# yvokeller/Show-Attend-and-Tell

Hardware: AMD Instinct MI355X
Metric: train images/sec on COCO batch=128 at 1/2/4/8 MI355X (higher is better)
Workload: dtype bf16; 1 GPU; COCO-shaped resnet152 encoder (bf16 fwd) + attention/tf/ado decoder train step, V=10000, T=27; global_batch=128, per_gpu_batch=128, seq_len=27, parallelism=dp1, hip_graph=True, encoder_decoder_overlap=True

## Files before the change

### include/sat_hip.h

```cpp
#ifndef SAT_HIP_H_
#define SAT_HIP_H_

#include <stddef.h>
#include <stdint.h>

#ifdef __cplusplus
extern "C" {
#endif

#define SAT_ABI_VERSION 9

enum { SAT_F32 = 0, SAT_BF16 = 1 };
enum { SAT_ACT_NONE = 0, SAT_ACT_RELU = 1, SAT_ACT_TANH = 2, SAT_ACT_SIGMOID = 3 };
enum { SAT_OK = 0, SAT_ERR_INVALID = 9001 };

typedef struct {
  int N, H, W, C, KH, KW, stride, pad, OH, OW;
} SatConvGeom;

typedef struct {
  int conv_pipe;
  int conv_stream;
  int conv3x3_ws;
  int conv_slices;
// ... 189 lines not shown
                            void* workspace, size_t workspace_bytes, int32_t* out_ids, int* out_len,
                            float* out_alphas, int* out_alpha_rows, float* out_score, void* stream);

size_t sat_decoder_beam_batch_workspace_bytes(const SatDecoderDims* d, int n_images, int beam_size, int max_step);
int sat_decoder_beam_search_batch(const SatDecoderDims* d, const SatDecoderLayout* lay, const float* params,
                                  const void* params_lp, const void* img_features, int n_images, int beam_size,
                                  int max_step, void* workspace, size_t workspace_bytes, int32_t* out_ids,
                                  int* out_len, float* out_alphas, int* out_alpha_rows, float* out_score,
                                  void* stream);

size_t sat_caption_loss_workspace_bytes(int B, int T, int L);
int sat_caption_loss_forward(int B, int T, int V, int L, int dtype, const void* preds,
                             const float* alphas, const int64_t* captions, float alpha_c,
                             int pad_id, int skip0, int skip1, int skip2, void* workspace,
                             float* out, void* stream);
int sat_caption_loss_forward_loss_out(int B, int T, int V, int L, int dtype, const void* preds,
                                      const float* alphas, const int64_t* captions, float alpha_c,
                                      int pad_id, int skip0, int skip1, int skip2, void* workspace,
                                      float* out, float* loss_out, void* stream);
int sat_caption_loss_backward(int B, int T, int V, int L, int dtype, const void* preds,
                              const int64_t* captions, float alpha_c, void* workspace,
                              const float* grad_out, void* d_preds, float* d_alphas, void* stream);
int sat_caption_loss_backward_relu(int B, int T, int V, int L, int dtype, const void* preds,
                              const int64_t* captions, float alpha_c, void* workspace,
                              const float* grad_out, void* d_preds, float* d_alphas, void* stream);
int sat_caption_loss_backward_ld(int B, int T, int V, int L, int dtype, const void* preds,
                                 const int64_t* captions, float alpha_c, void* workspace,
                                 const float* grad_out, void* d_preds, int64_t ld_dpreds,
                                 float* d_alphas, int relu_mask, void* stream);
size_t sat_caption_loss_weighted_workspace_bytes(int B, int T, int L);
int sat_caption_loss_weighted_forward(int B, int T, int V, int L, int dtype, const void* preds,
                                      const float* alphas, const int32_t* targets, const float* weights,
                                      float alpha_c, void* workspace, float* out, float* loss_out, float* logp,
                                      void* stream);
int sat_caption_loss_weighted_backward(int B, int T, int V, int L, int dtype, const void* preds,
                                       const int32_t* targets, const float* weights, void* workspace,
                                       const float* grad_out, void* d_preds, int64_t ld_dpreds, float* d_alphas,
                                       int relu_mask, void* stream);

enum { SAT_IMG_NCHW = 0, SAT_IMG_NHWC = 1, SAT_IMG_S2D16 = 2 };
size_t sat_images_workspace_bytes(int B, int OH, int OW);
int sat_images_max_downscale(void);
size_t sat_images_lds_bytes(int max_h, int max_w, int OH, int OW);
size_t sat_images_lds_limit(void);
int sat_images_to_input(const uint8_t* pixels, const int64_t* offsets, const int32_t* sizes, int B, int max_h,
                        int max_w, int OH, int OW, const float* mean, const float* std, int layout, int c_pad,
                        int dtype, void* out, void* workspace, size_t workspace_bytes, void* stream);

int sat_rows_gather(const void* table, int64_t n_rows, int64_t row_elems, int dtype, const int64_t* idx, int n,
                    void* out, int32_t* n_bad, void* stream);
int sat_rows_scatter(const void* src, int n, int64_t row_elems, int dtype, const int64_t* idx, void* table,
                     int64_t n_rows, int32_t* n_bad, void* stream);

int sat_cider_table_insert(uint32_t* table, int64_t slots, const uint32_t* keys, const float* values, int64_t n,
                           int32_t* n_bad, void* stream);
int sat_cider_lookup(const uint32_t* table, int64_t slots, float log_n, const uint32_t* keys, int64_t n, float* out,
                     void* stream);
int sat_cider_ref_norms(const uint32_t* table, int64_t slots, float log_n, const int32_t* ref_words,
                        const int32_t* ref_len, int n_refs, int ref_stride, float* ref_norm, void* stream);
int sat_cider_score(const uint32_t* table, int64_t slots, float log_n, const int32_t* ref_words,
                    const int32_t* ref_len, const float* ref_norm, int n_refs, int ref_stride,
                    const int32_t* img_ref_begin, int n_images, const int32_t* tokens, const int64_t* image, int n,
                    int T1, int start_id, int end_id, int pad_id, float* out, int32_t* n_bad, void* stream);

int sat_adam_step(float* param, const float* grad, float* exp_avg, float* exp_avg_sq,
                  void* param_lp, int64_t n, float beta1, float beta2, float eps,
                  float step_size, float bias_correction2_sqrt, void* stream);

#ifdef __cplusplus
}
#endif
#endif
```

### show-attend-and-tell_amd/_lib.py

```python
import ctypes
import os

import torch

_HERE = os.path.dirname(os.path.abspath(__file__))
LIB_PATH = os.environ.get("SAT_HIP_LIB_TUNING") or os.path.join(_HERE, "libsat_hip.so")

SAT_F32, SAT_BF16 = 0, 1
IMG_NCHW, IMG_NHWC, IMG_S2D16 = 0, 1, 2
ACT_NONE, ACT_RELU, ACT_TANH, ACT_SIGMOID = 0, 1, 2, 3

c_int, c_int64, c_float, c_void_p, c_size_t, c_uint64 = (ctypes.c_int, ctypes.c_int64, ctypes.c_float,
                                                        ctypes.c_void_p, ctypes.c_size_t, ctypes.c_uint64)


class SatConvGeom(ctypes.Structure):
    _fields_ = [(n, c_int) for n in ("N", "H", "W", "C", "KH", "KW", "stride", "pad", "OH", "OW")]


ABI_VERSION = 9


class SatPolicy(ctypes.Structure):
    _fields_ = [(n, c_int) for n in ("conv_pipe", "conv_stream", "conv3x3_ws", "conv_slices", "skinny", "gemm_stages",
# ... 137 lines not shown
    ("sat_decoder_forward_sample", c_int, [ctypes.POINTER(SatDecoderDims), ctypes.POINTER(SatDecoderLayout),
                                           c_void_p, c_void_p, c_void_p, c_void_p, c_void_p, c_float, c_void_p,
                                           c_void_p, c_size_t, c_void_p, c_void_p, c_void_p, c_void_p, c_void_p]),
    ("sat_sample_noise", c_int, [ctypes.POINTER(SatDecoderDims), c_int, c_int, c_int, c_void_p, c_void_p]),
    ("sat_decoder_backward", c_int, [ctypes.POINTER(SatDecoderDims), ctypes.POINTER(SatDecoderLayout), c_void_p,
                                     c_void_p, c_void_p, c_void_p, c_size_t, c_void_p, c_void_p, c_void_p,
                                     c_void_p, c_void_p, c_int, c_int, c_void_p]),
    ("sat_decoder_backward_features", c_int, [ctypes.POINTER(SatDecoderDims), ctypes.POINTER(SatDecoderLayout),
                                              c_void_p, c_void_p, c_void_p, c_void_p, c_size_t, c_void_p, c_void_p,
                                              c_void_p, c_void_p, c_void_p, c_int, c_int, c_void_p, c_void_p,
                                              c_void_p, c_size_t]),
    ("sat_decoder_feature_grad_workspace_bytes", c_size_t, [ctypes.POINTER(SatDecoderDims)]),
    ("sat_feature_grad_accumulate", c_int, [c_int, c_int, c_int, c_int, c_int, c_void_p, c_int64, c_int64, c_void_p,
                                            c_int64, c_int64, c_void_p, c_int64, c_void_p, c_int64, c_void_p,
                                            c_int64, c_void_p]),
    ("sat_decoder_step_bench", c_int, [ctypes.POINTER(SatDecoderDims), ctypes.POINTER(SatDecoderLayout), c_void_p,
                                       c_void_p, c_void_p, c_void_p, c_size_t, c_void_p, c_void_p, c_int, c_void_p,
                                       c_void_p]),
    ("sat_decoder_beam_workspace_bytes", c_size_t, [ctypes.POINTER(SatDecoderDims), c_int]),
    ("sat_decoder_beam_search", c_int, [ctypes.POINTER(SatDecoderDims), ctypes.POINTER(SatDecoderLayout), c_void_p,
                                        c_void_p, c_void_p, c_int, c_int, c_void_p, c_size_t, c_void_p, c_void_p,
                                        c_void_p, c_void_p, c_void_p, c_void_p]),
    ("sat_decoder_beam_batch_workspace_bytes", c_size_t, [ctypes.POINTER(SatDecoderDims), c_int, c_int, c_int]),
    ("sat_decoder_beam_search_batch", c_int, [ctypes.POINTER(SatDecoderDims), ctypes.POINTER(SatDecoderLayout),
                                              c_void_p, c_void_p, c_void_p, c_int, c_int, c_int, c_void_p, c_size_t,
                                              c_void_p, c_void_p, c_void_p, c_void_p, c_void_p, c_void_p]),
    ("sat_caption_loss_workspace_bytes", c_size_t, [c_int, c_int, c_int]),
    ("sat_caption_loss_forward", c_int, [c_int, c_int, c_int, c_int, c_int, c_void_p, c_void_p, c_void_p, c_float,
                                         c_int, c_int, c_int, c_int, c_void_p, c_void_p, c_void_p]),
    ("sat_caption_loss_forward_loss_out", c_int, [c_int, c_int, c_int, c_int, c_int, c_void_p, c_void_p, c_void_p,
                                                  c_float, c_int, c_int, c_int, c_int, c_void_p, c_void_p, c_void_p,
                                                  c_void_p]),
    ("sat_caption_loss_backward", c_int, [c_int, c_int, c_int, c_int, c_int, c_void_p, c_void_p, c_float,
                                          c_void_p, c_void_p, c_void_p, c_void_p, c_void_p]),
    ("sat_caption_loss_backward_relu", c_int, [c_int, c_int, c_int, c_int, c_int, c_void_p, c_void_p, c_float,
                                          c_void_p, c_void_p, c_void_p, c_void_p, c_void_p]),
    ("sat_caption_loss_backward_ld", c_int, [c_int, c_int, c_int, c_int, c_int, c_void_p, c_void_p, c_float,
                                             c_void_p, c_void_p, c_void_p, c_int64, c_void_p, c_int, c_void_p]),
    ("sat_caption_loss_weighted_workspace_bytes", c_size_t, [c_int, c_int, c_int]),
    ("sat_caption_loss_weighted_forward", c_int, [c_int, c_int, c_int, c_int, c_int, c_void_p, c_void_p, c_void_p,
                                                  c_void_p, c_float, c_void_p, c_void_p, c_void_p, c_void_p,
                                                  c_void_p]),
    ("sat_caption_loss_weighted_backward", c_int, [c_int, c_int, c_int, c_int, c_int, c_void_p, c_void_p, c_void_p,
                                                   c_void_p, c_void_p, c_void_p, c_int64, c_void_p, c_int, c_void_p]),
    ("sat_images_workspace_bytes", c_size_t, [c_int, c_int, c_int]),
    ("sat_images_max_downscale", c_int, []),
    ("sat_images_lds_bytes", c_size_t, [c_int, c_int, c_int, c_int]),
    ("sat_images_lds_limit", c_size_t, []),
    ("sat_images_to_input", c_int, [c_void_p, c_void_p, c_void_p, c_int, c_int, c_int, c_int, c_int,
                                    ctypes.POINTER(c_float), ctypes.POINTER(c_float), c_int, c_int, c_int, c_void_p,
                                    c_void_p, c_size_t, c_void_p]),
    ("sat_rows_gather", c_int, [c_void_p, c_int64, c_int64, c_int, c_void_p, c_int, c_void_p, c_void_p, c_void_p]),
    ("sat_rows_scatter", c_int, [c_void_p, c_int, c_int64, c_int, c_void_p, c_void_p, c_int64, c_void_p, c_void_p]),
    ("sat_cider_table_insert", c_int, [c_void_p, c_int64, c_void_p, c_void_p, c_int64, c_void_p, c_void_p]),
    ("sat_cider_lookup", c_int, [c_void_p, c_int64, c_float, c_void_p, c_int64, c_void_p, c_void_p]),
    ("sat_cider_ref_norms", c_int, [c_void_p, c_int64, c_float, c_void_p, c_void_p, c_int, c_int, c_void_p,
                                    c_void_p]),
    ("sat_cider_score", c_int, [c_void_p, c_int64, c_float, c_void_p, c_void_p, c_void_p, c_int, c_int, c_void_p,
                                c_int, c_void_p, c_void_p, c_int, c_int, c_int, c_int, c_int, c_void_p, c_void_p,
                                c_void_p]),
    ("sat_adam_step", c_int, [c_void_p, c_void_p, c_void_p, c_void_p, c_void_p, c_int64, c_float, c_float,
                              c_float, c_float, c_float, c_void_p]),
]
EXPORTED = [s[0] for s in _SIGNATURES]

_lib = None


def lib():
    global _lib
    if _lib is None:
        if not os.path.exists(LIB_PATH):
            raise RuntimeError(f"sat_amd: HIP library not found at {LIB_PATH}; build it with "
                               "`python -c 'import __graft_entry__ as g; g.build()'` (make -C "
                               "show-attend-and-tell_amd/csrc)")
        handle = ctypes.CDLL(LIB_PATH)
        for name, res, args in _SIGNATURES:
            fn = getattr(handle, name)
            fn.restype = res
            fn.argtypes = args
        version = handle.sat_abi_version()
        if version != ABI_VERSION:
            raise RuntimeError(f"sat_amd: {LIB_PATH} has C-ABI version {version}, this package binds version "
                               f"{ABI_VERSION}; rebuild it (make -C show-attend-and-tell_amd/csrc)")
        _lib = handle
    return _lib


def check(code, what):
    if code != 0:
        msg = lib().sat_error_string(code)
        raise RuntimeError(f"sat_amd: {what} failed with code {code}: {msg.decode() if msg else '?'}")


def dtype_code(dt):
    if dt == torch.float32:
        return SAT_F32
    if dt == torch.bfloat16:
        return SAT_BF16
    raise TypeError(f"sat_amd: unsupported dtype {dt} (float32 or bfloat16)")


def require_device(*tensors):
    for t in tensors:
        if t is not None and t.device.type != "cuda":
            raise RuntimeError("sat_amd: tensors must live on a HIP device (the product path has no CPU fallback)")
# ... 13 lines not shown
```

### show-attend-and-tell_amd/csrc/elementwise.hip

```cpp
#include "sat_common.h"
#include "sat_internal.h"

namespace {

constexpr int kMaxGrid = 2048;
inline int grid_for(long n, int per_block = 256) {
  long g = (n + per_block - 1) / per_block;
  return (int)(g < 1 ? 1 : (g > kMaxGrid ? kMaxGrid : g));
}

template <typename T>
__global__ void nchw_to_nhwc_kernel(const float* __restrict__ x, T* __restrict__ y, int N, int C, int H, int W,
                                    int Cp) {
  long total = (long)N * H * W;
  for (long p = blockIdx.x * (long)blockDim.x + threadIdx.x; p < total; p += (long)gridDim.x * blockDim.x) {
    long n = p / ((long)H * W), hw = p - n * H * W;
    const float* src = x + n * C * H * W + hw;
    T* dst = y + p * Cp;
    if (Cp * sizeof(T) == 16) {
      uint4 u;
      T* h = (T*)&u;
#pragma unroll
      for (int c = 0; c < 16 / (int)sizeof(T); ++c) h[c] = (T)(c < C ? src[(long)c * H * W] : 0.f);
      *(uint4*)dst = u;
// ... 356 lines not shown
      for (long i = blockIdx.x * (long)blockDim.x + threadIdx.x; i < R * C; i += stride) {
        const long r = i / C;
        p[r * ld + (i - r * C)] = 0.f;
      }
    }
  }
}

template <typename T>
__global__ void embed_gather_kernel(const float* __restrict__ W, const int32_t* __restrict__ tok, int R,
                                    long tok_stride_b, int T1, int E, T* __restrict__ out, long out_ld) {
  int r = blockIdx.x;
  if (r >= R) return;
  int b = r / T1, t = r - b * T1;
  int id = tok[(long)b * tok_stride_b + t];
  const float* src = W + (long)id * E;
  T* dst = out + (long)r * out_ld;
  for (int e = threadIdx.x; e < E; e += blockDim.x) dst[e] = (T)src[e];
}

template <typename OT>
__global__ void embed_gather_captions_kernel(const float* __restrict__ W, const int64_t* __restrict__ caps, int R,
                                             int T, int T1, int E, OT* __restrict__ out, long out_ld,
                                             int32_t* __restrict__ tok) {
  const int r = blockIdx.x;
  if (r >= R) return;
  const int b = r / T1, t = r - b * T1;
  const int id = (int)caps[(long)b * T + t];
  if (threadIdx.x == 0) tok[r] = id;
  const float* src = W + (long)id * E;
  OT* dst = out + (long)r * out_ld;
  if ((E & 3) == 0 && ((uintptr_t)src & 15) == 0) {
    for (int e = 4 * threadIdx.x; e < E; e += 4 * blockDim.x) {
      const float4 v = *(const float4*)(src + e);
      dst[e] = (OT)v.x; dst[e + 1] = (OT)v.y; dst[e + 2] = (OT)v.z; dst[e + 3] = (OT)v.w;
    }
  } else {
    for (int e = threadIdx.x; e < E; e += blockDim.x) dst[e] = (OT)src[e];
  }
}

__global__ void embed_scatter_kernel(const float* __restrict__ dX, const int32_t* __restrict__ tok, int R, int E,
                                     float* __restrict__ G) {
  int r = blockIdx.x;
  if (r >= R) return;
  int id = tok[r];
  const float* src = dX + (long)r * E;
  float* dst = G + (long)id * E;
  for (int e = threadIdx.x; e < E; e += blockDim.x) atomicAdd(dst + e, src[e]);
}

constexpr int kEmbSortMax = 16384, kEmbPiece = 32;
constexpr int kRankRows = 16, kRankParts = 16;
__global__ __launch_bounds__(256) void embed_rank_kernel(const int32_t* __restrict__ tok, int R,
                                                         int32_t* __restrict__ perm, int32_t* __restrict__ stok,
                                                         int32_t* __restrict__ seg) {
  __shared__ __attribute__((aligned(16))) int32_t st[kEmbSortMax];
  __shared__ int cnt[3][kRankParts][kRankRows];
  const int R4 = (R + 3) & ~3;
  for (int i = threadIdx.x; i < R4; i += blockDim.x) st[i] = i < R ? tok[i] : 0x7fffffff;
  __syncthreads();
  const int rl = threadIdx.x & (kRankRows - 1), part = threadIdx.x / kRankRows;
  const int r = blockIdx.x * kRankRows + rl;
  const int k = r < R ? st[r] : 0;
  const int words = R4 / 4, per = (words + kRankParts - 1) / kRankParts;
  const int w0 = part * per, w1 = min(words, w0 + per);
  int less = 0, before = 0, eq = 0;
#pragma unroll 4
  for (int wi = w0; wi < w1; ++wi) {
    const int i = 4 * wi;
    const int4 x = *(const int4*)(st + i);
    less += (x.x < k) + (x.y < k) + (x.z < k) + (x.w < k);
    eq += (x.x == k) + (x.y == k) + (x.z == k) + (x.w == k);
    before += ((x.x == k) & (i < r)) + ((x.y == k) & (i + 1 < r)) + ((x.z == k) & (i + 2 < r)) + ((x.w == k) & (i + 3 < r));
  }
  cnt[0][part][rl] = less; cnt[1][part][rl] = eq; cnt[2][part][rl] = before;
  __syncthreads();
  if (part != 0 || r >= R) return;
  for (int q = 1; q < kRankParts; ++q) { less += cnt[0][q][rl]; eq += cnt[1][q][rl]; before += cnt[2][q][rl]; }
  const int pos = less + before;
  perm[pos] = r;
  stok[pos] = k;
  seg[2 * pos] = less;
  seg[2 * pos + 1] = less + eq;
}

__global__ __launch_bounds__(64) void embed_segsum_kernel(const float* __restrict__ dX, int E,
                                                          const int32_t* __restrict__ perm,
                                                          const int32_t* __restrict__ stok,
                                                          const int32_t* __restrict__ seg, int R, float* G,
                                                          float* __restrict__ part, int accumulate) {
  const int p = blockIdx.x, e = blockIdx.y * 256 + 4 * threadIdx.x;
  const int s0 = p * kEmbPiece, n = min(R - s0, kEmbPiece);
  __shared__ int sr[kEmbPiece], stk[kEmbPiece], sa[kEmbPiece], sb[kEmbPiece];
  if ((int)threadIdx.x < n) {
    sr[threadIdx.x] = perm[s0 + threadIdx.x];
    stk[threadIdx.x] = stok[s0 + threadIdx.x];
    sa[threadIdx.x] = seg[2 * (s0 + threadIdx.x)];
    sb[threadIdx.x] = seg[2 * (s0 + threadIdx.x) + 1];
  }
  __syncthreads();
  if (e >= E) return;
  float4 x[kEmbPiece];
#pragma unroll
  for (int i = 0; i < kEmbPiece; ++i)
    x[i] = i < n ? *(const float4*)(dX + (long)sr[i] * E + e) : make_float4(0.f, 0.f, 0.f, 0.f);
  float4 acc = make_float4(0.f, 0.f, 0.f, 0.f);
  int rs = 0;
#pragma unroll
  for (int i = 0; i < kEmbPiece; ++i) {
    if (i < n) {
      acc = f4add(acc, x[i]);
      if (i + 1 == n || stk[i + 1] != stk[i]) {
        if (sa[i] == s0 + rs && sb[i] == s0 + i + 1) {
          float4* g = (float4*)(G + (long)stk[i] * E + e);
          *g = accumulate ? f4add(*g, acc) : acc;
        } else {
          *(float4*)(part + ((long)p * 2 + (rs == 0 ? 0 : 1)) * E + e) = acc;
        }
        acc = make_float4(0.f, 0.f, 0.f, 0.f);
        rs = i + 1;
      }
    }
  }
}

__global__ __launch_bounds__(256) void embed_segfix_kernel(const int32_t* __restrict__ stok,
                                                           const int32_t* __restrict__ seg, int R, int E,
                                                           const float* __restrict__ part, float* G,
                                                           int accumulate) {
  const int p = blockIdx.x, chain = threadIdx.x >> 6, e = blockIdx.y * 256 + 4 * (threadIdx.x & 63);
  const int s0 = p * kEmbPiece, s1 = min(R, s0 + kEmbPiece);
  const int sa = seg[2 * (s1 - 1)], sb = seg[2 * (s1 - 1) + 1];
  if (sb <= s1 || sa < s0) return;
  __shared__ float4 cs[3][64];
  const int p1 = (sb - 1) / kEmbPiece;
  float4 acc = make_float4(0.f, 0.f, 0.f, 0.f);
  if (e < E) {
    for (int q0 = p + 1 + chain; q0 <= p1; q0 += 32) {
      float4 y[8];
#pragma unroll
      for (int u = 0; u < 8; ++u) {
        const int q = q0 + 4 * u;
        y[u] = q <= p1 ? *(const float4*)(part + (long)q * 2 * E + e) : make_float4(0.f, 0.f, 0.f, 0.f);
      }
#pragma unroll
      for (int u = 0; u < 8; ++u) acc = f4add(acc, y[u]);
    }
  }
  if (chain > 0) cs[chain - 1][threadIdx.x & 63] = acc;
  __syncthreads();
  if (chain != 0 || e >= E) return;
  const float4 own = *(const float4*)(part + ((long)p * 2 + (sa == s0 ? 0 : 1)) * E + e);
  const float4 sum = f4add(own, f4add(f4add(acc, cs[0][threadIdx.x]), f4add(cs[1][threadIdx.x], cs[2][threadIdx.x])));
  float4* g = (float4*)(G + (long)stok[s1 - 1] * E + e);
  *g = accumulate ? f4add(*g, sum) : sum;
}

__device__ __forceinline__ bool am_better(float x, int xi, float y, int yi) { return sat_argmax_better(x, xi, y, yi); }
// ... 288 lines not shown
    else hipLaunchKernelGGL((argmax_kernel<bf16, false, true>), dim3(B), dim3(256), 0, s, (const bf16*)X, ld, V, out, out_stride, emb, E, (bf16*)emb_out, emb_ld, pre, pre_stride);
  } else {
    if (vec) hipLaunchKernelGGL((argmax_kernel<float, true, true>), dim3(B), dim3(256), 0, s, (const float*)X, ld, V, out, out_stride, emb, E, (float*)emb_out, emb_ld, pre, pre_stride);
    else hipLaunchKernelGGL((argmax_kernel<float, false, true>), dim3(B), dim3(256), 0, s, (const float*)X, ld, V, out, out_stride, emb, E, (float*)emb_out, emb_ld, pre, pre_stride);
  }
  return (int)hipGetLastError();
}

int sat_argmax_rows_sample(const void* X, int dtype, long ld, int B, int V, int32_t* out, long out_stride,
                           int32_t* out2, long out2_stride, const float* emb, int E, void* emb_out, long emb_ld,
                           const SatSampleArgs& sa, hipStream_t s) {
  if (V >= (1 << 20) || sa.t < 0 || sa.t >= (1 << 20)) return (int)hipErrorInvalidValue;
  const int esz = dtype == SAT_BF16 ? 2 : 4;
  const bool vec = ((uintptr_t)X & 15) == 0 && (ld * esz) % 16 == 0;
  if (dtype == SAT_BF16) {
    if (vec) hipLaunchKernelGGL((argmax_kernel<bf16, true, false, true>), dim3(B), dim3(256), 0, s, (const bf16*)X, ld, V, out, out_stride, emb, E, (bf16*)emb_out, emb_ld, nullptr, 0, sa, out2, out2_stride);
    else hipLaunchKernelGGL((argmax_kernel<bf16, false, false, true>), dim3(B), dim3(256), 0, s, (const bf16*)X, ld, V, out, out_stride, emb, E, (bf16*)emb_out, emb_ld, nullptr, 0, sa, out2, out2_stride);
  } else {
    if (vec) hipLaunchKernelGGL((argmax_kernel<float, true, false, true>), dim3(B), dim3(256), 0, s, (const float*)X, ld, V, out, out_stride, emb, E, (float*)emb_out, emb_ld, nullptr, 0, sa, out2, out2_stride);
    else hipLaunchKernelGGL((argmax_kernel<float, false, false, true>), dim3(B), dim3(256), 0, s, (const float*)X, ld, V, out, out_stride, emb, E, (float*)emb_out, emb_ld, nullptr, 0, sa, out2, out2_stride);
  }
  return (int)hipGetLastError();
}

int sat_cast_launch(const void* x, int xd, void* y, int yd, long n, hipStream_t s) {
  if (n <= 0) return 0;
  int g = grid_for(n);
  if (xd == SAT_F32 && yd == SAT_BF16) hipLaunchKernelGGL((cast_kernel<float, bf16>), dim3(g), dim3(256), 0, s, (const float*)x, (bf16*)y, n);
  else if (xd == SAT_BF16 && yd == SAT_F32) hipLaunchKernelGGL((cast_kernel<bf16, float>), dim3(g), dim3(256), 0, s, (const bf16*)x, (float*)y, n);
  else if (xd == SAT_F32) hipLaunchKernelGGL((cast_kernel<float, float>), dim3(g), dim3(256), 0, s, (const float*)x, (float*)y, n);
  else hipLaunchKernelGGL((cast_kernel<bf16, bf16>), dim3(g), dim3(256), 0, s, (const bf16*)x, (bf16*)y, n);
  return (int)hipGetLastError();
}

extern "C" int sat_abi_version(void) { return SAT_ABI_VERSION; }

extern "C" const char* sat_error_string(int code) {
  if (code == 0) return "success";
  if (code == SAT_ERR_INVALID) return "invalid argument or unsupported shape";
  return hipGetErrorString((hipError_t)code);
}

extern "C" int sat_cast(const void* x, int x_dtype, void* y, int y_dtype, int64_t n, void* stream) {
  SAT_REQUIRE(x && y && n >= 0);
  return sat_cast_launch(x, x_dtype, y, y_dtype, n, (hipStream_t)stream);
}

extern "C" int sat_mean_rows_abi(const void* a, int B, int L, int D, int dtype, float* out_f32, void* out_t,
                                 void* stream) {
  SAT_REQUIRE(a && B > 0 && L > 0 && D > 0);
  return sat_mean_rows(a, B, L, D, dtype, out_f32, out_t, (hipStream_t)stream);
}

extern "C" int sat_nchw_to_nhwc(int N, int C, int H, int W, int Cp, int dtype, const float* x, void* y,
                                void* stream) {
  SAT_REQUIRE(x && y && Cp >= C && C > 0);
  long pix = (long)N * H * W;
  int g = grid_for(pix);
  if (dtype == SAT_BF16)
    hipLaunchKernelGGL(nchw_to_nhwc_kernel<bf16>, dim3(g), dim3(256), 0, (hipStream_t)stream, x, (bf16*)y, N, C, H, W, Cp);
  else
    hipLaunchKernelGGL(nchw_to_nhwc_kernel<float>, dim3(g), dim3(256), 0, (hipStream_t)stream, x, (float*)y, N, C, H, W, Cp);
  return (int)hipGetLastError();
}

extern "C" int sat_nchw_to_s2d(int N, int C, int H, int W, int dtype, const float* x, void* y, void* stream) {
  SAT_REQUIRE(x && y && C > 0 && 4 * C <= 16 && H % 2 == 0 && W % 2 == 0);
  const int g = grid_for((long)N * (H / 2) * (W / 2));
  if (dtype == SAT_BF16 && C == 3 && ((uintptr_t)x & 7) == 0 && ((uintptr_t)y & 15) == 0) {
    const long total = (long)N * (H / 2) * (W / 2);
    hipLaunchKernelGGL(nchw3_to_s2d16_bf16_kernel, dim3((unsigned)((total + 255) / 256)), dim3(256), 0,
                       (hipStream_t)stream, x, (bf16*)y, N, H, W);
  } else if (dtype == SAT_BF16)
    hipLaunchKernelGGL(nchw_to_s2d16_kernel<bf16>, dim3(g), dim3(256), 0, (hipStream_t)stream, x, (bf16*)y, N, C, H, W);
  else
    hipLaunchKernelGGL(nchw_to_s2d16_kernel<float>, dim3(g), dim3(256), 0, (hipStream_t)stream, x, (float*)y, N, C, H, W);
  return (int)hipGetLastError();
}

extern "C" int sat_maxpool2d_nhwc(int N, int H, int W, int C, int k, int stride, int pad, int dtype, const void* x,
                                  void* y, int OH, int OW, void* stream) {
  SAT_REQUIRE(x && y && k > 0 && stride > 0);
  SAT_REQUIRE(OH == (H + 2 * pad - k) / stride + 1 && OW == (W + 2 * pad - k) / stride + 1);
  SAT_REQUIRE(C % 8 == 0 && ((uintptr_t)x & 15) == 0 && ((uintptr_t)y & 15) == 0);
  long total = (long)N * OH * OW * (C / 8);
  int g = grid_for(total);
  if (dtype == SAT_BF16 && k == 3) {
    hipLaunchKernelGGL(maxpool_bf16_kernel<3>, dim3((unsigned)((total + 255) / 256)), dim3(256), 0,
                       (hipStream_t)stream, (const bf16*)x, (bf16*)y, N, H, W, C, stride, pad, OH, OW);
  } else if (dtype == SAT_BF16)
    hipLaunchKernelGGL(maxpool_kernel<bf16>, dim3(g), dim3(256), 0, (hipStream_t)stream, (const bf16*)x, (bf16*)y, N, H,
                       W, C, k, stride, pad, OH, OW);
  else
    hipLaunchKernelGGL(maxpool_kernel<float>, dim3(g), dim3(256), 0, (hipStream_t)stream, (const float*)x, (float*)y, N,
                       H, W, C, k, stride, pad, OH, OW);
  return (int)hipGetLastError();
}

extern "C" int sat_adam_step(float* param, const float* grad, float* exp_avg, float* exp_avg_sq, void* param_lp,
                             int64_t n, float beta1, float beta2, float eps, float step_size,
                             float bias_correction2_sqrt, void* stream) {
  SAT_REQUIRE(param && grad && exp_avg && exp_avg_sq && n >= 0);
  constexpr int64_t kChunk = 1L << 28;
  for (int64_t i = 0; i < n; i += kChunk) {
    const int64_t m = n - i < kChunk ? n - i : kChunk;
    hipLaunchKernelGGL(adam_kernel, dim3(grid_for((m + 3) / 4)), dim3(256), 0, (hipStream_t)stream, param + i, grad + i,
// ... 7 lines not shown
```

### show-attend-and-tell_amd/csrc/loss.hip

```cpp
#include "sat_common.h"
#include "sat_internal.h"

namespace {

constexpr int kStat = 5;

__device__ __forceinline__ float block_sum(float v, float* red) {
  const int lane = threadIdx.x & 63, w = threadIdx.x >> 6, nw = blockDim.x >> 6;
  v = wave_sum(v);
  __syncthreads();
  if (lane == 0) red[w] = v;
  __syncthreads();
  float s = 0.f;
  for (int i = 0; i < nw; ++i) s += red[i];
  return s;
}
__device__ __forceinline__ float block_max(float v, float* red) {
  const int lane = threadIdx.x & 63, w = threadIdx.x >> 6, nw = blockDim.x >> 6;
  v = wave_max(v);
  __syncthreads();
  if (lane == 0) red[w] = v;
  __syncthreads();
  float s = -INFINITY;
  for (int i = 0; i < nw; ++i) s = fmaxf(s, red[i]);
// ... 147 lines not shown
    constexpr int LU = 4;
    const int NV = V / VEC;
    for (int c0 = threadIdx.x; c0 < NV; c0 += LU * 256) {
      uint4 u[LU];
#pragma unroll
      for (int k = 0; k < LU; ++k) {
        const int c = c0 + k * 256;
        u[k] = c < NV ? *(const uint4*)(x + (long)c * VEC) : make_uint4(0u, 0u, 0u, 0u);
      }
#pragma unroll
      for (int k = 0; k < LU; ++k) {
        const int c = c0 + k * 256;
        if (c >= NV) break;
        const TT* h = (const TT*)&u[k];
#pragma unroll
        for (int j = 0; j < VEC; ++j) {
          const float xv = (float)h[j];
          const int v = c * VEC + j;
          online_add(m, se, xv);
          cnt += (xv > xt || (xv == xt && v < tgt)) ? 1.f : 0.f;
        }
      }
    }
  } else {
    for (int v = threadIdx.x; v < V; v += blockDim.x) {
      const float xv = (float)x[v];
      online_add(m, se, xv);
      cnt += (xv > xt || (xv == xt && v < tgt)) ? 1.f : 0.f;
    }
  }
#pragma unroll
  for (int o = 32; o > 0; o >>= 1) {
    const float om = __shfl_xor(m, o, 64), os = __shfl_xor(se, o, 64);
    const float nm = fmaxf(m, om);
    se = (nm == -INFINITY) ? 0.f : se * expf(m - nm) + os * expf(om - nm);
    m = nm;
    cnt += __shfl_xor(cnt, o, 64);
  }
  const int lane = threadIdx.x & 63, w = threadIdx.x >> 6;
  if (lane == 0) { red_m[w] = m; red_s[w] = se; red_c[w] = cnt; }
  __syncthreads();
  if (threadIdx.x == 0) {
    float M = red_m[0], S = red_s[0], C = red_c[0];
    for (int i = 1; i < 4; ++i) {
      const float nm = fmaxf(M, red_m[i]);
      S = (nm == -INFINITY) ? 0.f : S * expf(M - nm) + red_s[i] * expf(red_m[i] - nm);
      M = nm;
      C += red_c[i];
    }
    write_stats(M + logf(S), xt, C);
  }
}

__global__ __launch_bounds__(256) void loss_reg_kernel(const float* __restrict__ alphas, int B, int T1, int L,
                                                       float alpha_c, float* __restrict__ dreg,
                                                       float* __restrict__ part) {
  __shared__ float red[4];
  const int i = blockIdx.x * blockDim.x + threadIdx.x;
  const float inv_bl = 1.0f / (float)(B * L);
  float reg = 0.f;
  if (i < B * L) {
    const int b = i / L, l = i - b * L;
    float ssum = 0.f;
    for (int t = 0; t < T1; ++t) ssum += alphas[((long)b * T1 + t) * L + l];
    const float d = 1.f - ssum;
    reg = d * d;
    dreg[i] = alpha_c * 2.f * (ssum - 1.f) * inv_bl;
  }
  reg = block_sum(reg, red);
  if (threadIdx.x == 0) part[blockIdx.x] = reg;
}

__global__ __launch_bounds__(1024) void loss_reduce_kernel(const float* __restrict__ stats, const float* __restrict__ part,
                                                           int nparts, const int64_t* __restrict__ caps, int B, int T,
                                                           int L, float alpha_c, int s0, int s1, int s2,
                                                           float* __restrict__ out, float* __restrict__ loss_out) {
  __shared__ float red[16];
  const int T1 = T - 1, R = B * T1;
  float ce = 0.f, c1 = 0.f, c5 = 0.f, np = 0.f;
  for (int r = threadIdx.x; r < R; r += blockDim.x) {
    const float* st = stats + (long)r * kStat;
    ce += st[1]; c1 += st[2]; c5 += st[3]; np += st[4];
  }
  ce = block_sum(ce, red);
  c1 = block_sum(c1, red);
  c5 = block_sum(c5, red);
  np = block_sum(np, red);
  float reg = 0.f;
  for (int i = threadIdx.x; i < nparts; i += blockDim.x) reg += part[i];
  reg = block_sum(reg, red);
  float cl = 0.f;
  for (int i = threadIdx.x; i < B * T; i += blockDim.x) {
    const int64_t tok = caps[i];
    cl += (tok != s0 && tok != s1 && tok != s2) ? 1.f : 0.f;
  }
  cl = block_sum(cl, red);
  if (threadIdx.x == 0) {
    const float cem = ce / (float)(B * (T1 - 1));
    const float regm = alpha_c * (reg * (1.0f / (float)(B * L)));
    out[0] = cem + regm;
    if (loss_out) loss_out[0] = cem + regm;
    out[1] = cem;
    out[2] = regm;
    out[3] = c1; out[4] = c5; out[5] = np; out[6] = cl;
  }
}

__global__ __launch_bounds__(1024) void wloss_reduce_kernel(const float* __restrict__ stats, const float* __restrict__ part,
                                                            int nparts, int R, int BL, float alpha_c,
                                                            float* __restrict__ out, float* __restrict__ loss_out) {
  __shared__ float red[16];
  float ce = 0.f, bad = 0.f;
  for (int r = threadIdx.x; r < R; r += blockDim.x) {
    const float* st = stats + (long)r * kStat;
    ce += st[1]; bad += st[2];
  }
  ce = block_sum(ce, red);
  bad = block_sum(bad, red);
  float reg = 0.f;
  for (int i = threadIdx.x; i < nparts; i += blockDim.x) reg += part[i];
  reg = block_sum(reg, red);
  if (threadIdx.x == 0) {
    const float regm = alpha_c * (reg * (1.0f / (float)BL));
    out[0] = ce + regm;
    loss_out[0] = ce + regm;
    out[1] = ce;
    out[2] = regm;
    out[3] = bad;
  }
}

template <typename TT, bool MASK, bool WT = false>
__global__ __launch_bounds__(256) void loss_bwd_kernel(const TT* __restrict__ preds, const int64_t* __restrict__ caps,
                                                       int B, int T, int V, int L, const float* __restrict__ stats,
                                                       const float* __restrict__ dreg, const float* __restrict__ grad_out,
                                                       TT* __restrict__ dpreds, long ldo, float* __restrict__ dalphas,
                                                       WArgs wa = WArgs{}) {
  const int r = blockIdx.x;
  const int T1 = T - 1;
  const int b = r / T1, t = r - b * T1;
  const float g = grad_out ? grad_out[0] : 1.f;
  const TT* x = preds + (long)r * V;
  TT* dx = dpreds + (long)r * ldo;
  bool scored;
  int tgt;
  float scale;
  if constexpr (WT) {
    tgt = wa.target[r];
    const float w = (tgt >= 0 && tgt < V) ? wa.w[r] : 0.f;
    scored = w != 0.f;
    scale = g * w;
  } else {
    scored = t < T1 - 1;
    tgt = scored ? (int)caps[(long)b * T + t + 1] : -1;
    scale = scored ? g / (float)(B * (T1 - 1)) : 0.f;
  }
  const float lse = scored ? stats[(long)r * kStat] : 0.f;
  auto grad = [&](float xv, int v) {
    float p = scored ? expf(xv - lse) : 0.f;
    if (v == tgt) p -= 1.f;
    float d = p * scale;
    if (MASK && !(xv > 0.f)) d = 0.f;
    return d;
  };
  constexpr int VEC = 16 / sizeof(TT);
  if (WT && !scored) {
    if (ldo % VEC == 0 && ((uintptr_t)dpreds & 15) == 0)
      for (long c = threadIdx.x; c < ldo / VEC; c += blockDim.x) *(uint4*)(dx + c * VEC) = make_uint4(0u, 0u, 0u, 0u);
    else
      for (long v = threadIdx.x; v < ldo; v += blockDim.x) dx[v] = (TT)0.f;
  } else if (V % VEC == 0 && ldo % VEC == 0) {
    const __amdgpu_buffer_rsrc_t rdx = sat_out_rsrc(dx, (long)sizeof(TT) * V);
    constexpr int LU = 4;
// ... 215 lines not shown
```

### show-attend-and-tell_amd/ops.py

```python
import ctypes

import torch

from . import _lib as L


def linear(x, weight, bias=None, act=L.ACT_NONE, out_dtype=None, weight_lp=None):
    L.require_device(x, weight)
    M, K = x.shape
    N = weight.shape[0]
    dt = L.dtype_code(x.dtype)
    if dt == L.SAT_F32:
        w = weight
    elif weight_lp is not None:
        w = weight_lp
    else:
        w = cast_(weight.contiguous(), torch.empty(weight.shape, device=weight.device, dtype=torch.bfloat16))
    out_dtype = out_dtype or torch.float32
    y = torch.empty(M, N, device=x.device, dtype=out_dtype)
    gemm(x, w, y, bias=bias, act=act)
    return y


_GEMM_WS = {}
# ... 368 lines not shown
    return out


def maxpool2d_nhwc(x, k, stride, pad=0):
    L.require_device(x)
    N, H, W, C = x.shape
    OH = (H + 2 * pad - k) // stride + 1
    OW = (W + 2 * pad - k) // stride + 1
    y = torch.empty(N, OH, OW, C, device=x.device, dtype=x.dtype)
    L.check(L.lib().sat_maxpool2d_nhwc(N, H, W, C, k, stride, pad, L.dtype_code(x.dtype), L.ptr(x), L.ptr(y), OH, OW,
                                       L.stream_of(y)), "sat_maxpool2d_nhwc")
    return y


def _rows_args(what, table, idx, batch, n_bad):
    L.require_device(table, idx, batch, n_bad)
    if table.dim() < 1 or table.shape[0] == 0 or not table.is_contiguous():
        raise ValueError(f"{what}: table must be a contiguous [n_rows, ...] tensor with n_rows > 0")
    if idx.dtype != torch.int64 or idx.dim() != 1 or not idx.is_contiguous():
        raise ValueError(f"{what}: idx must be a contiguous int64 vector")
    if batch.dtype != table.dtype or tuple(batch.shape) != (idx.shape[0],) + tuple(table.shape[1:]) \
            or not batch.is_contiguous():
        raise ValueError(f"{what}: expected a contiguous {table.dtype} batch of shape "
                         f"{(idx.shape[0],) + tuple(table.shape[1:])}, got {batch.dtype} {tuple(batch.shape)}")
    if n_bad is not None and (n_bad.dtype != torch.int32 or n_bad.numel() != 1):
        raise ValueError(f"{what}: n_bad must be one int32")
    row_elems = table.numel() // table.shape[0]
    if row_elems == 0:
        raise ValueError(f"{what}: empty rows")
    return table.shape[0], row_elems


def rows_gather(table, idx, out=None, n_bad=None):
    if out is None:
        L.require_device(table, idx)
        out = torch.empty((idx.shape[0],) + tuple(table.shape[1:]), device=table.device, dtype=table.dtype)
    n_rows, row_elems = _rows_args("rows_gather", table, idx, out, n_bad)
    if idx.shape[0] == 0:
        return out
    L.check(L.lib().sat_rows_gather(L.ptr(table), n_rows, row_elems, L.dtype_code(table.dtype), L.ptr(idx),
                                    idx.shape[0], L.ptr(out), L.ptr(n_bad), L.stream_of(out)), "sat_rows_gather")
    return out


def rows_scatter(src, idx, table, n_bad=None):
    n_rows, row_elems = _rows_args("rows_scatter", table, idx, src, n_bad)
    if idx.shape[0] == 0:
        return table
    L.check(L.lib().sat_rows_scatter(L.ptr(src), idx.shape[0], row_elems, L.dtype_code(table.dtype), L.ptr(idx),
                                     L.ptr(table), n_rows, L.ptr(n_bad), L.stream_of(table)), "sat_rows_scatter")
    return table


CIDER_MAX_WORDS = 64
CIDER_ID_LIMIT = 1 << 20


def _cider_table_args(what, table):
    L.require_device(table)
    if table.dtype != torch.int32 or table.dim() != 2 or table.shape[1] != 4 or table.shape[0] < 2 \
            or not table.is_contiguous():
        raise ValueError(f"{what}: table must be a contiguous int32 [slots, 4] tensor with slots >= 2")
    return table.shape[0]


def _cider_keys_args(what, table, keys, other, other_dtype):
    L.require_device(keys, other)
    if keys.dtype != torch.int32 or keys.dim() != 2 or keys.shape[1] != 3 or not keys.is_contiguous() \
            or keys.device != table.device:
        raise ValueError(f"{what}: keys must be a contiguous int32 [n, 3] tensor on the table's device")
    if other.dtype != other_dtype or tuple(other.shape) != (keys.shape[0],) or not other.is_contiguous():
        raise ValueError(f"{what}: expected a contiguous {other_dtype} vector of {keys.shape[0]} elements")


def cider_table_insert(table, keys, values, n_bad=None):
    slots = _cider_table_args("cider_table_insert", table)
    _cider_keys_args("cider_table_insert", table, keys, values, torch.float32)
    L.require_device(n_bad)
    if n_bad is not None and (n_bad.dtype != torch.int32 or n_bad.numel() != 1):
        raise ValueError("cider_table_insert: n_bad must be one int32")
    if keys.shape[0]:
        L.check(L.lib().sat_cider_table_insert(L.ptr(table), slots, L.ptr(keys), L.ptr(values), keys.shape[0],
                                               L.ptr(n_bad), L.stream_of(table)), "sat_cider_table_insert")
    return table


def cider_lookup(table, log_n, keys, out=None):
    slots = _cider_table_args("cider_lookup", table)
    if out is None:
        L.require_device(keys)
        out = torch.empty(keys.shape[0], device=keys.device, dtype=torch.float32)
    _cider_keys_args("cider_lookup", table, keys, out, torch.float32)
    if keys.shape[0]:
        L.check(L.lib().sat_cider_lookup(L.ptr(table), slots, float(log_n), L.ptr(keys), keys.shape[0], L.ptr(out),
                                         L.stream_of(out)), "sat_cider_lookup")
    return out


def _cider_refs_args(what, table, ref_words, ref_len, ref_norm):
    L.require_device(ref_words, ref_len, ref_norm)
    n_refs = ref_len.shape[0] if ref_len.dim() == 1 else -1
    if ref_words.dtype != torch.int32 or ref_words.dim() != 2 or not ref_words.is_contiguous() \
            or ref_words.shape[0] < max(1, n_refs) or not 1 <= ref_words.shape[1] <= CIDER_MAX_WORDS:
        raise ValueError(f"{what}: ref_words must be a contiguous int32 [n_refs, stride <= {CIDER_MAX_WORDS}] tensor")
    if ref_len.dtype != torch.int32 or n_refs < 0 or not ref_len.is_contiguous():
        raise ValueError(f"{what}: ref_len must be a contiguous int32 vector")
# ... 55 lines not shown
```

Measured before the change: 22810 images/s.

## Batch loads in embed rank, scatter-add and loss reduction kernels; expose sorted embed ABI

The embed rank kernel now fills shared memory with vectorized int4 loads, unrolled several per thread. The sorted scatter-add kernel loads every row slot unconditionally, with indices clamped, and hoists row pointers into scalar registers via readfirstlane. The loss reg and reduce kernels switch to unrolled batched loads so more memory requests are in flight. A new exported ABI and Python wrapper for the sorted embedding scatter-add is also added. These are small kernels, so the effect on end-to-end training throughput should be minor.

New measurement: 22850 images/s (median of 6 runs). Within noise of the previous version (+0.2%).

```diff
diff --git a/include/sat_hip.h b/include/sat_hip.h
--- a/include/sat_hip.h
+++ b/include/sat_hip.h
@@ -265,6 +265,11 @@
 int sat_rows_scatter(const void* src, int n, int64_t row_elems, int dtype, const int64_t* idx, void* table,
                      int64_t n_rows, int32_t* n_bad, void* stream);
 
+int sat_embed_sorted_max_rows_abi(void);
+size_t sat_embed_sorted_workspace_bytes(int R, int E);
+int sat_embed_scatter_add_sorted_ws(const float* dX, const int32_t* tok, int R, int E, float* G, int accumulate,
+                                    void* workspace, size_t workspace_bytes, void* stream);
+
 int sat_cider_table_insert(uint32_t* table, int64_t slots, const uint32_t* keys, const float* values, int64_t n,
                            int32_t* n_bad, void* stream);
 int sat_cider_lookup(const uint32_t* table, int64_t slots, float log_n, const uint32_t* keys, int64_t n, float* out,
diff --git a/show-attend-and-tell_amd/_lib.py b/show-attend-and-tell_amd/_lib.py
--- a/show-attend-and-tell_amd/_lib.py
+++ b/show-attend-and-tell_amd/_lib.py
@@ -213,6 +213,10 @@
                                     c_void_p, c_size_t, c_void_p]),
     ("sat_rows_gather", c_int, [c_void_p, c_int64, c_int64, c_int, c_void_p, c_int, c_void_p, c_void_p, c_void_p]),
     ("sat_rows_scatter", c_int, [c_void_p, c_int, c_int64, c_int, c_void_p, c_void_p, c_int64, c_void_p, c_void_p]),
+    ("sat_embed_sorted_max_rows_abi", c_int, []),
+    ("sat_embed_sorted_workspace_bytes", c_size_t, [c_int, c_int]),
+    ("sat_embed_scatter_add_sorted_ws", c_int, [c_void_p, c_void_p, c_int, c_int, c_void_p, c_int, c_void_p, c_size_t,
+                                                c_void_p]),
     ("sat_cider_table_insert", c_int, [c_void_p, c_int64, c_void_p, c_void_p, c_int64, c_void_p, c_void_p]),
     ("sat_cider_lookup", c_int, [c_void_p, c_int64, c_float, c_void_p, c_int64, c_void_p, c_void_p]),
     ("sat_cider_ref_norms", c_int, [c_void_p, c_int64, c_float, c_void_p, c_void_p, c_int, c_int, c_void_p,
diff --git a/show-attend-and-tell_amd/csrc/elementwise.hip b/show-attend-and-tell_amd/csrc/elementwise.hip
--- a/show-attend-and-tell_amd/csrc/elementwise.hip
+++ b/show-attend-and-tell_amd/csrc/elementwise.hip
@@ -432,13 +432,39 @@
 
 constexpr int kEmbSortMax = 16384, kEmbPiece = 32;
 constexpr int kRankRows = 16, kRankParts = 16;
+constexpr int kRankLoad = 4;
 __global__ __launch_bounds__(256) void embed_rank_kernel(const int32_t* __restrict__ tok, int R,
                                                          int32_t* __restrict__ perm, int32_t* __restrict__ stok,
                                                          int32_t* __restrict__ seg) {
   __shared__ __attribute__((aligned(16))) int32_t st[kEmbSortMax];
   __shared__ int cnt[3][kRankParts][kRankRows];
   const int R4 = (R + 3) & ~3;
-  for (int i = threadIdx.x; i < R4; i += blockDim.x) st[i] = i < R ? tok[i] : 0x7fffffff;
+  constexpr int kThreads = kRankRows * kRankParts;
+  const int tid = threadIdx.x;
+  if (((uintptr_t)tok & 15) == 0) {
+    const int nfull = R >> 2;
+    const int ti = min(4 * nfull + (tid & 3), R4 - 1);
+    const int32_t tl = tok[min(ti, R - 1)];
+    for (int base = 0; base < nfull; base += kThreads * kRankLoad) {
+      int4 v[kRankLoad];
+#pragma unroll
+      for (int u = 0; u < kRankLoad; ++u) v[u] = *(const int4*)(tok + 4 * min(base + u * kThreads + tid, nfull - 1));
+#pragma unroll
+      for (int u = 0; u < kRankLoad; ++u) *(int4*)(st + 4 * min(base + u * kThreads + tid, nfull - 1)) = v[u];
+    }
+    st[ti] = ti < R ? tl : 0x7fffffff;
+  } else {
+    for (int base = 0; base < R4; base += kThreads * kRankLoad) {
+      int32_t v[kRankLoad];
+#pragma unroll
+      for (int u = 0; u < kRankLoad; ++u) v[u] = tok[min(base + u * kThreads + tid, R - 1)];
+#pragma unroll
+      for (int u = 0; u < kRankLoad; ++u) {
+        const int i = min(base + u * kThreads + tid, R4 - 1);
+        st[i] = i < R ? v[u] : 0x7fffffff;
+      }
+    }
+  }
   __syncthreads();
   const int rl = threadIdx.x & (kRankRows - 1), part = threadIdx.x / kRankRows;
   const int r = blockIdx.x * kRankRows + rl;
@@ -472,19 +498,24 @@
                                                           float* __restrict__ part, int accumulate) {
   const int p = blockIdx.x, e = blockIdx.y * 256 + 4 * threadIdx.x;
   const int s0 = p * kEmbPiece, n = min(R - s0, kEmbPiece);
-  __shared__ int sr[kEmbPiece], stk[kEmbPiece], sa[kEmbPiece], sb[kEmbPiece];
-  if ((int)threadIdx.x < n) {
-    sr[threadIdx.x] = perm[s0 + threadIdx.x];
-    stk[threadIdx.x] = stok[s0 + threadIdx.x];
-    sa[threadIdx.x] = seg[2 * (s0 + threadIdx.x)];
-    sb[threadIdx.x] = seg[2 * (s0 + threadIdx.x) + 1];
+  __shared__ __attribute__((aligned(16))) int sr[kEmbPiece];
+  __shared__ int stk[kEmbPiece], sa[kEmbPiece], sb[kEmbPiece];
+  if ((int)threadIdx.x < kEmbPiece) {
+    const int s = s0 + min((int)threadIdx.x, n - 1);
+    sr[threadIdx.x] = perm[s];
+    stk[threadIdx.x] = stok[s];
+    sa[threadIdx.x] = seg[2 * s];
+    sb[threadIdx.x] = seg[2 * s + 1];
   }
   __syncthreads();
   if (e >= E) return;
+  const float* src[kEmbPiece];
+#pragma unroll
+  for (int i = 0; i < kEmbPiece; ++i)
+    src[i] = dX + (long)__builtin_amdgcn_readfirstlane(sr[i]) * E;
   float4 x[kEmbPiece];
 #pragma unroll
-  for (int i = 0; i < kEmbPiece; ++i)
-    x[i] = i < n ? *(const float4*)(dX + (long)sr[i] * E + e) : make_float4(0.f, 0.f, 0.f, 0.f);
+  for (int i = 0; i < kEmbPiece; ++i) x[i] = *(const float4*)(src[i] + e);
   float4 acc = make_float4(0.f, 0.f, 0.f, 0.f);
   int rs = 0;
 #pragma unroll
@@ -879,6 +910,19 @@
   return sat_mean_rows(a, B, L, D, dtype, out_f32, out_t, (hipStream_t)stream);
 }
 
+extern "C" int sat_embed_sorted_max_rows_abi(void) { return sat_embed_sorted_max_rows(); }
+extern "C" size_t sat_embed_sorted_workspace_bytes(int R, int E) {
+  return R > 0 && E > 0 ? sat_embed_sorted_ws_bytes(R, E) : 0;
+}
+extern "C" int sat_embed_scatter_add_sorted_ws(const float* dX, const int32_t* tok, int R, int E, float* G,
+                                               int accumulate, void* workspace, size_t workspace_bytes, void* stream) {
+  SAT_REQUIRE(R >= 0 && E > 0 && E % 4 == 0 && R <= sat_embed_sorted_max_rows());
+  if (R == 0) return 0;
+  SAT_REQUIRE(dX && tok && G && workspace && ((uintptr_t)dX & 15) == 0 && ((uintptr_t)G & 15) == 0 &&
+              ((uintptr_t)workspace & 15) == 0 && workspace_bytes >= sat_embed_sorted_ws_bytes(R, E));
+  return sat_embed_scatter_add_sorted(dX, tok, R, E, G, accumulate, workspace, (hipStream_t)stream);
+}
+
 extern "C" int sat_nchw_to_nhwc(int N, int C, int H, int W, int Cp, int dtype, const float* x, void* y,
                                 void* stream) {
   SAT_REQUIRE(x && y && Cp >= C && C > 0);
diff --git a/show-attend-and-tell_amd/csrc/loss.hip b/show-attend-and-tell_amd/csrc/loss.hip
--- a/show-attend-and-tell_amd/csrc/loss.hip
+++ b/show-attend-and-tell_amd/csrc/loss.hip
@@ -223,6 +223,7 @@
   }
 }
 
+constexpr int kRegLoad = 16;
 __global__ __launch_bounds__(256) void loss_reg_kernel(const float* __restrict__ alphas, int B, int T1, int L,
                                                        float alpha_c, float* __restrict__ dreg,
                                                        float* __restrict__ part) {
@@ -232,14 +233,39 @@
   float reg = 0.f;
   if (i < B * L) {
     const int b = i / L, l = i - b * L;
+    const float* col = alphas + (long)b * T1 * L + l;
     float ssum = 0.f;
-    for (int t = 0; t < T1; ++t) ssum += alphas[((long)b * T1 + t) * L + l];
+    for (int t0 = 0; t0 < T1; t0 += kRegLoad) {
+      float v[kRegLoad];
+#pragma unroll
+      for (int u = 0; u < kRegLoad; ++u) v[u] = col[(long)min(t0 + u, T1 - 1) * L];
+#pragma unroll
+      for (int u = 0; u < kRegLoad; ++u)
+        if (t0 + u < T1) ssum += v[u];
+    }
     const float d = 1.f - ssum;
     reg = d * d;
     dreg[i] = alpha_c * 2.f * (ssum - 1.f) * inv_bl;
   }
   reg = block_sum(reg, red);
   if (threadIdx.x == 0) part[blockIdx.x] = reg;
+}
+
+constexpr int kRedLoad = 4;
+template <typename V>
+__device__ __forceinline__ void load_strided(const V* __restrict__ p, int n, int base, V (&v)[kRedLoad]) {
+#pragma unroll
+  for (int u = 0; u < kRedLoad; ++u) v[u] = p[min(base + u * (int)blockDim.x + (int)threadIdx.x, n - 1)];
+}
+template <int C0, int NC>
+__device__ __forceinline__ void load_stat_rows(const float* __restrict__ stats, int R, int base,
+                                               float (&v)[kRedLoad][NC]) {
+#pragma unroll
+  for (int u = 0; u < kRedLoad; ++u) {
+    const float* st = stats + (long)min(base + u * (int)blockDim.x + (int)threadIdx.x, R - 1) * kStat + C0;
+#pragma unroll
+    for (int c = 0; c < NC; ++c) v[u][c] = st[c];
+  }
 }
 
 __global__ __launch_bounds__(1024) void loss_reduce_kernel(const float* __restrict__ stats, const float* __restrict__ part,
@@ -247,23 +273,41 @@
                                                            int L, float alpha_c, int s0, int s1, int s2,
                                                            float* __restrict__ out, float* __restrict__ loss_out) {
   __shared__ float red[16];
-  const int T1 = T - 1, R = B * T1;
+  const int T1 = T - 1, R = B * T1, BT = B * T;
+  float sv[kRedLoad][4], pv[kRedLoad];
+  int64_t cv[kRedLoad];
+  load_stat_rows<1, 4>(stats, R, 0, sv);
+  load_strided(part, nparts, 0, pv);
+  load_strided(caps, BT, 0, cv);
+  const int step = kRedLoad * blockDim.x;
   float ce = 0.f, c1 = 0.f, c5 = 0.f, np = 0.f;
-  for (int r = threadIdx.x; r < R; r += blockDim.x) {
-    const float* st = stats + (long)r * kStat;
-    ce += st[1]; c1 += st[2]; c5 += st[3]; np += st[4];
+  for (int base = 0; base < R; base += step) {
+    if (base) load_stat_rows<1, 4>(stats, R, base, sv);
+#pragma unroll
+    for (int u = 0; u < kRedLoad; ++u)
+      if (base + u * (int)blockDim.x + (int)threadIdx.x < R) { ce += sv[u][0]; c1 += sv[u][1]; c5 += sv[u][2]; np += sv[u][3]; }
   }
   ce = block_sum(ce, red);
   c1 = block_sum(c1, red);
   c5 = block_sum(c5, red);
   np = block_sum(np, red);
   float reg = 0.f;
-  for (int i = threadIdx.x; i < nparts; i += blockDim.x) reg += part[i];
+  for (int base = 0; base < nparts; base += step) {
+    if (base) load_strided(part, nparts, base, pv);
+#pragma unroll
+    for (int u = 0; u < kRedLoad; ++u)
+      if (base + u * (int)blockDim.x + (int)threadIdx.x < nparts) reg += pv[u];
+  }
   reg = block_sum(reg, red);
   float cl = 0.f;
-  for (int i = threadIdx.x; i < B * T; i += blockDim.x) {
-    const int64_t tok = caps[i];
-    cl += (tok != s0 && tok != s1 && tok != s2) ? 1.f : 0.f;
+  for (int base = 0; base < BT; base += step) {
+    if (base) load_strided(caps, BT, base, cv);
+#pragma unroll
+    for (int u = 0; u < kRedLoad; ++u)
+      if (base + u * (int)blockDim.x + (int)threadIdx.x < BT) {
+        const int64_t tok = cv[u];
+        cl += (tok != s0 && tok != s1 && tok != s2) ? 1.f : 0.f;
+      }
   }
   cl = block_sum(cl, red);
   if (threadIdx.x == 0) {
@@ -281,15 +325,26 @@
                                                             int nparts, int R, int BL, float alpha_c,
                                                             float* __restrict__ out, float* __restrict__ loss_out) {
   __shared__ float red[16];
+  float sv[kRedLoad][2], pv[kRedLoad];
+  load_stat_rows<1, 2>(stats, R, 0, sv);
+  load_strided(part, nparts, 0, pv);
+  const int step = kRedLoad * blockDim.x;
   float ce = 0.f, bad = 0.f;
-  for (int r = threadIdx.x; r < R; r += blockDim.x) {
-    const float* st = stats + (long)r * kStat;
-    ce += st[1]; bad += st[2];
+  for (int base = 0; base < R; base += step) {
+    if (base) load_stat_rows<1, 2>(stats, R, base, sv);
+#pragma unroll
+    for (int u = 0; u < kRedLoad; ++u)
+      if (base + u * (int)blockDim.x + (int)threadIdx.x < R) { ce += sv[u][0]; bad += sv[u][1]; }
   }
   ce = block_sum(ce, red);
   bad = block_sum(bad, red);
   float reg = 0.f;
-  for (int i = threadIdx.x; i < nparts; i += blockDim.x) reg += part[i];
+  for (int base = 0; base < nparts; base += step) {
+    if (base) load_strided(part, nparts, base, pv);
+#pragma unroll
+    for (int u = 0; u < kRedLoad; ++u)
+      if (base + u * (int)blockDim.x + (int)threadIdx.x < nparts) reg += pv[u];
+  }
   reg = block_sum(reg, red);
   if (threadIdx.x == 0) {
     const float regm = alpha_c * (reg * (1.0f / (float)BL));
diff --git a/show-attend-and-tell_amd/ops.py b/show-attend-and-tell_amd/ops.py
--- a/show-attend-and-tell_amd/ops.py
+++ b/show-attend-and-tell_amd/ops.py
@@ -444,6 +444,28 @@
     return table
 
 
+def embed_scatter_add_sorted(dX, tok, G, accumulate=True):
+    L.require_device(dX, tok, G)
+    if dX.dtype != torch.float32 or dX.dim() != 2 or not dX.is_contiguous():
+        raise ValueError("embed_scatter_add_sorted: dX must be a contiguous fp32 [R, E] tensor")
+    R, E = dX.shape
+    if G.dtype != torch.float32 or G.dim() != 2 or G.shape[1] != E or G.shape[0] == 0 or not G.is_contiguous():
+        raise ValueError(f"embed_scatter_add_sorted: G must be a contiguous fp32 [V, {E}] tensor")
+    if tok.dtype != torch.int32 or tuple(tok.shape) != (R,) or not tok.is_contiguous():
+        raise ValueError(f"embed_scatter_add_sorted: tok must be a contiguous int32 vector of {R} tokens")
+    lib = L.lib()
+    if E == 0 or E % 4 or R > lib.sat_embed_sorted_max_rows_abi():
+        raise ValueError(f"embed_scatter_add_sorted: E % 4 == 0 and R <= {lib.sat_embed_sorted_max_rows_abi()} "
+                         f"required, got R = {R}, E = {E}")
+    if R == 0:
+        return G
+    nbytes = lib.sat_embed_sorted_workspace_bytes(R, E)
+    ws = torch.empty(nbytes, device=dX.device, dtype=torch.uint8)
+    L.check(lib.sat_embed_scatter_add_sorted_ws(L.ptr(dX), L.ptr(tok), R, E, L.ptr(G), int(bool(accumulate)),
+                                                L.ptr(ws), nbytes, L.stream_of(G)), "sat_embed_scatter_add_sorted_ws")
+    return G
+
+
 CIDER_MAX_WORDS = 64
 CIDER_ID_LIMIT = 1 << 20
 
```
